# spcl/gemm_hls

Measured on AMD Instinct MI355X. Metric: GFLOP/s, fp32 GEMM N=K=M=16384 per MI355X (tiled outer-product C=A.B), and % of fp32 MFMA peak, higher is better.
Workload: dtype f32; 1 GPU; float 16384x16384x16384 (Multiply,Add) on 1 MI355X; BASELINE configs[1]; kernel=mfma_f32_256x256x16_w8_flush4096, rows_total=16384, rows_per_gpu=16384

## Files before the change

gemm_hls_amd/csrc/mm_capi.hip:

```cpp
#include <algorithm>
#include <atomic>
#include <chrono>
#include <cstdarg>
#include <cstdio>
#include <cstdlib>
#include <cstring>
#include <mutex>
#include <random>
#include <unordered_map>
#include <vector>

#include "mm_common.h"

namespace {

thread_local char g_error[512] = "";

int fail(int code, const char *fmt, ...) {
  va_list ap;
  va_start(ap, fmt);
  vsnprintf(g_error, sizeof(g_error), fmt, ap);
  va_end(ap);
  return code;
}
// ... 6 lines not shown
#define MM_HIP(call)                                   \
  do {                                                 \
    hipError_t e_ = (call);                            \
    if (e_ != hipSuccess) return hip_fail(e_, #call);  \
  } while (0)

std::once_flag g_init_once;
int g_device_count = 0;
int g_device_cus[64] = {};
int g_init_status = MM_ERR_NO_DEVICE;
char g_init_error[512] = "";

void init_once() {
  auto init_fail = [](const char *fmt, auto... args) {
    snprintf(g_init_error, sizeof(g_init_error), fmt, args...);
    g_device_count = 0;
    g_init_status = MM_ERR_NO_DEVICE;
  };
  int n = 0;
  hipError_t e = hipGetDeviceCount(&n);
  if (e != hipSuccess || n <= 0)
    return init_fail("hipGetDeviceCount: %s; this library needs an MI355X (gfx950), there is no CPU fallback",
                     e == hipSuccess ? "0 devices" : hipGetErrorString(e));
  for (int d = 0; d < n; ++d) {
    hipDeviceProp_t prop;
    e = hipGetDeviceProperties(&prop, d);
    if (e != hipSuccess) return init_fail("hipGetDeviceProperties(%d): %s", d, hipGetErrorString(e));
    if (strncmp(prop.gcnArchName, "gfx950", 6) != 0)
      return init_fail("device %d is %s; the kernels in this library are built for gfx950 only "
                       "(hide other devices with HIP_VISIBLE_DEVICES)", d, prop.gcnArchName);
    if (d < 64) g_device_cus[d] = prop.multiProcessorCount;
  }
  g_device_count = n;
  g_init_status = MM_OK;
}

int ensure_init() {
  std::call_once(g_init_once, init_once);
  return g_init_status == MM_OK ? MM_OK : fail(g_init_status, "%s", g_init_error);
}

std::mutex g_default_cfg_mutex;
mm_config_t g_default_cfg = {MM_DTYPE_F32, MM_OP_MULTIPLY, MM_OP_ADD, MM_PATH_AUTO, MM_A_ROW_MAJOR};
mm_config_t default_cfg() {
  std::lock_guard<std::mutex> lock(g_default_cfg_mutex);
  return g_default_cfg;
}

std::once_flag g_tuning_once;
std::atomic<int> g_tuning[mm::TUNE_COUNT];
const char *const kTuneName[mm::TUNE_COUNT] = {"f32_variant", "f64_variant", "f16_variant", "i8_variant", "band_rows",
                                               "valu_variant", "split_variant", "f32_splitk", "ablations", "debug_poison", "kxn_prepass_min_m",
                                               "md_virtual_devices", "ordered_variant", "half_contract", "batch_chunk",
                                               "closure_block", "lse_variant"};
const char *const kTuneEnv[mm::TUNE_COUNT] = {"MM_F32_VARIANT", "MM_F64_VARIANT", "MM_F16_VARIANT", "MM_I8_VARIANT",
                                              "MM_BAND_ROWS", "MM_VALU_VARIANT", "MM_SPLIT_VARIANT", "MM_F32_SPLITK", "MM_ABLATIONS", "MM_DEBUG_POISON", "MM_KXN_PREPASS_MIN_M",
                                              "MM_MD_VIRTUAL_DEVICES", "MM_ORDERED_VARIANT", "MM_HALF_CONTRACT", "MM_BATCH_CHUNK",
                                              "MM_CLOSURE_BLOCK", "MM_LSE_VARIANT"};
void tuning_init() {
  for (int i = 0; i < mm::TUNE_COUNT; ++i) {
    const char *e = getenv(kTuneEnv[i]);
    int v = (e && *e) ? atoi(e) : -1;
    if (i == mm::TUNE_HALF_CONTRACT && e && *e) {
      if (strcmp(e, "reference") == 0) v = 1;
      else if (strcmp(e, "wide") == 0) v = 0;
    }
    g_tuning[i].store(v, std::memory_order_relaxed);
  }
}

int check_device(int device) {
  int rc = ensure_init();
  if (rc) return rc;
  if (device < 0 || device >= g_device_count)
    return fail(MM_ERR_BAD_ARGUMENT, "device %d out of range [0, %d)", device, g_device_count);
  return MM_OK;
}

bool valid_cfg(const mm_config_t *cfg) {
  return cfg && cfg->dtype >= MM_DTYPE_F32 && cfg->dtype <= MM_DTYPE_U64 && cfg->map_op >= MM_OP_ADD &&
         cfg->map_op <= MM_OP_MAX && cfg->reduce_op >= MM_OP_ADD && cfg->reduce_op <= MM_OP_MAX &&
         (cfg->path == MM_PATH_AUTO || cfg->path == MM_PATH_ORDERED || cfg->path == MM_PATH_SPLIT) &&
         (cfg->layout_a == MM_A_ROW_MAJOR || cfg->layout_a == MM_A_TRANSPOSED);
}

int f32_variant() { return mm::tuning(mm::TUNE_F32_VARIANT); }
int f32_variant_for(const mm::Problem &p) { return mm::mfma_f32_resolve(p, f32_variant()); }

enum Family { FAM_ORDERED, FAM_ORDERED_TILE, FAM_VALU_TILE, FAM_MFMA_F32, FAM_MFMA_F64, FAM_MFMA_F16, FAM_MFMA_I8, FAM_HALF_WIDE,
              FAM_F32_SPLIT, FAM_NONE };

Family choose(const mm_config_t &cfg, const mm::Problem &slab) {
  mm::Problem p = slab;
  if (slab.n_total) { p.n = slab.n_total; p.n_total = 0; }
  const bool mul_add = cfg.map_op == MM_OP_MULTIPLY && cfg.reduce_op == MM_OP_ADD;
  const bool reference_half = cfg.path == MM_PATH_AUTO && mul_add && cfg.dtype == MM_DTYPE_F16 && mm::tuning(mm::TUNE_HALF_CONTRACT) == 1;
  if (cfg.path == MM_PATH_ORDERED || reference_half)
    return mm::tuning(mm::TUNE_ORDERED_VARIANT) != 0 && mm::valu_tile_serves(cfg, p) ? FAM_ORDERED_TILE : FAM_ORDERED;
  if (cfg.path == MM_PATH_SPLIT)
    return mul_add && cfg.dtype == MM_DTYPE_F32 && mm::mfma_f32_split_serves(p) ? FAM_F32_SPLIT : FAM_NONE;
  if (mul_add && cfg.dtype == MM_DTYPE_F32 && mm::mfma_f32_serves(p)) return FAM_MFMA_F32;
  if (mul_add && cfg.dtype == MM_DTYPE_F64 && mm::mfma_f64_serves(p)) return FAM_MFMA_F64;
  if (mul_add && cfg.dtype == MM_DTYPE_F16) return mm::mfma_f16_serves(p) ? FAM_MFMA_F16 : FAM_HALF_WIDE;
  if (mul_add && (cfg.dtype == MM_DTYPE_I8 || cfg.dtype == MM_DTYPE_U8) && mm::mfma_i8_serves(p)) return FAM_MFMA_I8;
  return mm::valu_tile_serves(cfg, p) ? FAM_VALU_TILE : FAM_ORDERED;
}

bool aligned16(const mm::Problem &p) {
  return (((uintptr_t)p.a | (uintptr_t)p.b | (uintptr_t)p.c) & 15u) == 0;
}

// ... 1478 lines not shown
```

gemm_hls_amd/csrc/mm_common.h:

```cpp
#pragma once
#include <hip/hip_runtime.h>
#include <stdint.h>
#include <stdlib.h>

#include <type_traits>

#include "../../include/mm_gemm.h"

namespace mm {

using half_t = _Float16;

template <typename T> struct Limits;
template <> struct Limits<float> {
  __host__ __device__ static constexpr float max() { return 3.40282346638528859812e+38f; }
  __host__ __device__ static constexpr float lowest() { return -3.40282346638528859812e+38f; }
};
template <> struct Limits<double> {
  __host__ __device__ static constexpr double max() { return 1.79769313486231570815e+308; }
  __host__ __device__ static constexpr double lowest() { return -1.79769313486231570815e+308; }
};
template <> struct Limits<half_t> {
  __host__ __device__ static constexpr half_t max() { return (half_t)65504.0f; }
  __host__ __device__ static constexpr half_t lowest() { return (half_t)-65504.0f; }
// ... 208 lines not shown
  switch (op) {
#define MM_CASE(OP) \
  case OP:          \
    if constexpr (OPS::template has<OP>) return f(std::integral_constant<int, OP>{}); else break;
    MM_CASE(MM_OP_ADD)
    MM_CASE(MM_OP_MULTIPLY)
    MM_CASE(MM_OP_AND)
    MM_CASE(MM_OP_MIN)
    MM_CASE(MM_OP_MAX)
#undef MM_CASE
  }
  return kErrNotSupported;
}

template <typename TYPES, typename MAPS, typename REDS, typename Fn>
int switch_config(const mm_config_t &cfg, Fn f) {
  return switch_dtype<TYPES>(cfg.dtype, [&](auto t) {
    return switch_op<MAPS>(cfg.map_op, [&](auto map) {
      return switch_op<REDS>(cfg.reduce_op, [&](auto red) { return f(t, map, red); });
    });
  });
}

inline int ensure_dynamic_lds(const void *func, int bytes, unsigned long long &mask) {
  int dev = 0;
  hipError_t e = hipGetDevice(&dev);
  if (e != hipSuccess) return (int)e;
  const unsigned long long bit = 1ull << (dev & 63);
  if (__atomic_load_n(&mask, __ATOMIC_ACQUIRE) & bit) return 0;
  e = hipFuncSetAttribute(func, hipFuncAttributeMaxDynamicSharedMemorySize, bytes);
  if (e != hipSuccess) return (int)e;
  __atomic_fetch_or(&mask, bit, __ATOMIC_RELEASE);
  return 0;
}

enum Tunable {
  TUNE_F32_VARIANT = 0,
  TUNE_F64_VARIANT,
  TUNE_F16_VARIANT,
  TUNE_I8_VARIANT,
  TUNE_BAND_ROWS,
  TUNE_VALU_VARIANT,
  TUNE_SPLIT_VARIANT,
  TUNE_F32_SPLITK,
  TUNE_ABLATIONS,
  TUNE_DEBUG_POISON,
  TUNE_KXN_PREPASS_MIN_M,
  TUNE_MD_VIRTUAL_DEVICES,
  TUNE_ORDERED_VARIANT,
  TUNE_HALF_CONTRACT,
  TUNE_BATCH_CHUNK,
  TUNE_CLOSURE_BLOCK,
  TUNE_LSE_VARIANT,
  TUNE_COUNT
};
int tuning(Tunable t);

inline unsigned band_rows(unsigned bm = 256, unsigned bn = 256, unsigned per_cu = 1) {
  const int v = tuning(TUNE_BAND_ROWS);
  if (v > 0) return (unsigned)v;
  const unsigned t = 32u * per_cu;
  unsigned best = 4, cost = ~0u;
  for (unsigned r = 1; r <= t; r *= 2) {
    const unsigned c = r * bm + (t / r) * bn;
    if (c < cost) { cost = c; best = r; }
  }
  return best;
}

struct TileCandidate { int id; unsigned bm, bn, per_cu; double eff; };
inline int pick_tile(const TileCandidate *cands, int count, unsigned n, unsigned m, double *best_time = nullptr,
                     unsigned long long copies = 1) {
  double best = 0;
  int pick = cands[0].id;
  for (int i = 0; i < count; ++i) {
    const TileCandidate &c = cands[i];
    const unsigned long long tiles = (unsigned long long)((n + c.bm - 1) / c.bm) * ((m + c.bn - 1) / c.bn) * copies;
    const unsigned long long slots = 256ull * c.per_cu, full = tiles / slots, rem = tiles % slots;
    const double t = ((double)full * c.per_cu + (double)((rem + 255) / 256)) * c.bm * c.bn / c.eff;
    if (best == 0 || t < best * 0.999) { best = t; pick = c.id; }
  }
  if (best_time) *best_time = best;
  return pick;
}

__device__ __forceinline__ unsigned xcd_remap(unsigned bid, unsigned nwg) {
  constexpr unsigned kXcds = 8;
  const unsigned q = nwg / kXcds, r = nwg % kXcds;
  const unsigned xcd = bid % kXcds, slot = bid / kXcds;
  const unsigned base = xcd < r ? xcd * (q + 1) : r * (q + 1) + (xcd - r) * q;
  return base + slot;
}

enum class Form { Single, Batched, Seeded };

template <Form F, typename G, auto KERN, typename T, typename CT>
int launch_tile(hipStream_t s, const Problem &p) {
  const unsigned tiles_n = (p.n + G::BM - 1) / G::BM, tiles_m = (p.m + G::BN - 1) / G::BN;
  static unsigned long long configured = 0;
  if (int e = ensure_dynamic_lds((const void *)KERN, G::LDS_BYTES, configured)) return e;
  hipLaunchKernelGGL(KERN, dim3(tiles_n * tiles_m * (F == Form::Single ? 1u : p.batch)), dim3(G::THREADS), G::LDS_BYTES, s,
                     (const T *)p.a, (const T *)p.b, (CT *)p.c, p.n, p.k, p.m, tiles_n, tiles_m, band_rows(G::BM, G::BN, 1),
                     F == Form::Single ? 1u : p.batch, p.stride_a, p.stride_b, p.stride_c);
  return (int)hipGetLastError();
}

// ... 64 lines not shown
```

gemm_hls_amd/csrc/mm_mfma_f32.hip:

```cpp
#include <cstdlib>
#include <type_traits>

#include "mm_common.h"

namespace mm {
namespace {

#include "mm_mfma_f32_tile.inc"
#include "mm_mfma_f32_small.inc"
#include "mm_mfma_f32_streamk.inc"

__global__ __launch_bounds__(256) void splitk_reduce_kernel(const float *__restrict__ partials, float *__restrict__ C,
                                                            size_t quads, unsigned splits) {
  const size_t i = (size_t)blockIdx.x * 256 + threadIdx.x;
  if (i >= quads) return;
  const f32x4 *src = (const f32x4 *)partials;
  f32x4 acc = src[i];
  for (unsigned s = 1; s < splits; ++s) acc += src[(size_t)s * quads + i];
  ((f32x4 *)C)[i] = acc;
}

template <typename G, bool AT = false>
int launch_geo(hipStream_t s, const Problem &p, unsigned splits = 1) {
  const unsigned tiles_n = (p.n + G::BM - 1) / G::BM, tiles_m = (p.m + G::BN - 1) / G::BN;
  static unsigned long long configured = 0;
  if (int e = ensure_dynamic_lds((const void *)mfma_f32_kernel<G, AT>, G::LDS_BYTES, configured)) return e;
  (void)hipGetLastError();
  if (splits <= 1) {
    hipLaunchKernelGGL((mfma_f32_kernel<G, AT>), dim3(tiles_n * tiles_m), dim3(G::THREADS), G::LDS_BYTES, s,
                       (const float *)p.a, (const float *)p.b, (float *)p.c, p.n, p.k, p.m, tiles_n, tiles_m,
                       band_rows(G::BM, G::BN, G::MIN_WAVES), 0u, (float *)nullptr);
    return (int)hipGetLastError();
  }
  const unsigned chunk = ((p.k + splits - 1) / splits + 31u) & ~31u;
  const size_t plane = (size_t)p.n * p.m;
  int dev = 0;
  hipError_t e = hipGetDevice(&dev);
  if (e != hipSuccess) return (int)e;
  hipMemPool_t pool = nullptr;
  if (int rc = workspace_pool(dev, &pool)) return rc;
  float *ws = nullptr;
  if ((e = hipMallocFromPoolAsync((void **)&ws, plane * splits * sizeof(float), pool, s)) != hipSuccess) return (int)e;
  hipLaunchKernelGGL((mfma_f32_kernel<G, AT>), dim3(tiles_n * tiles_m * splits), dim3(G::THREADS), G::LDS_BYTES, s,
                     (const float *)p.a, (const float *)p.b, (float *)p.c, p.n, p.k, p.m, tiles_n, tiles_m,
                     band_rows(G::BM, G::BN, G::MIN_WAVES), chunk, ws);
  int rc = (int)hipGetLastError();
  if (rc == 0) {
    const size_t quads = plane / 4;
    hipLaunchKernelGGL(splitk_reduce_kernel, dim3((unsigned)((quads + 255) / 256)), dim3(256), 0, s, ws, (float *)p.c, quads, splits);
    rc = (int)hipGetLastError();
  }
  const hipError_t f = hipFreeAsync(ws, s);
  return rc ? rc : (int)f;
}

template <typename G, bool AT, bool SEED>
__global__ __launch_bounds__(G::THREADS, G::MIN_WAVES) void mfma_f32_batched_kernel(
    const float *__restrict__ A, const float *__restrict__ B, float *__restrict__ C, unsigned N, unsigned K, unsigned M,
    unsigned tiles_n, unsigned tiles_m, unsigned kBand, unsigned batch, size_t stride_a, size_t stride_b, size_t stride_c) {
  const unsigned lin = batched_tile(A, B, C, tiles_n * tiles_m, batch, stride_a, stride_b, stride_c);
  const unsigned band = lin / (kBand * tiles_m), within = lin % (kBand * tiles_m);
  const unsigned rows_in_band = min(kBand, tiles_n - band * kBand);
  const unsigned tile_row = band * kBand + within % rows_in_band;
  const unsigned tile_col = within / rows_in_band;
  tile_body<G, AT, false, SEED>(A, B, C, N, K, M, K, M, N, M, tile_row * G::BM, tile_col * G::BN);
}

template <typename G, bool AT, bool SEED>
int launch_geo_batched_seed(hipStream_t s, const Problem &p) {
  const unsigned tiles_n = (p.n + G::BM - 1) / G::BM, tiles_m = (p.m + G::BN - 1) / G::BN;
  static unsigned long long configured = 0;
  (void)hipGetLastError();
  if (int e = ensure_dynamic_lds((const void *)mfma_f32_batched_kernel<G, AT, SEED>, G::LDS_BYTES, configured)) return e;
  hipLaunchKernelGGL((mfma_f32_batched_kernel<G, AT, SEED>), dim3(tiles_n * tiles_m * p.batch), dim3(G::THREADS), G::LDS_BYTES,
                     s, (const float *)p.a, (const float *)p.b, (float *)p.c, p.n, p.k, p.m, tiles_n, tiles_m,
                     band_rows(G::BM, G::BN, G::MIN_WAVES), p.batch, p.stride_a, p.stride_b, p.stride_c);
  return (int)hipGetLastError();
}

template <typename G, bool AT = false>
int launch_geo_batched(hipStream_t s, const Problem &p) {
  return p.seed ? launch_geo_batched_seed<G, AT, true>(s, p) : launch_geo_batched_seed<G, AT, false>(s, p);
}

using T128x256 = Geo<2, 2, 2, 16, Chain::FlushIntoC, 256, Reads::Pipelined, Dma::ScalarBase>;
using T128x256v = Geo<2, 2, 2, 16, Chain::FlushIntoC, 256, Reads::Pipelined, Dma::VectorAddress>;
using T256x256 = Geo<2, 4, 2, 16, Chain::FlushIntoC, 256, Reads::Pipelined, Dma::ScalarBase>;
using T256x256v = Geo<2, 4, 2, 16, Chain::FlushIntoC, 256, Reads::Pipelined, Dma::VectorAddress>;
using T128x128 = Geo<1, 4, 1, 32, Chain::FlushIntoC, 128, Reads::Pipelined, Dma::ScalarBase>;
using T128x128v = Geo<1, 4, 1, 32, Chain::FlushIntoC, 128, Reads::Pipelined, Dma::VectorAddress>;
using X128x256x32_2lvl = Geo<2, 2, 2, 32, Chain::TwoLevel, 16, Reads::CompilerPlaced, Dma::VectorAddress>;
using X256x256_single = Geo<2, 4, 2, 16, Chain::Single, 1, Reads::CompilerPlaced, Dma::VectorAddress>;

struct VariantInfo { int id; const char *name; unsigned bm, bn, bk, waves; };
template <typename G> constexpr VariantInfo info_of(int id, const char *name) { return {id, name, G::BM, G::BN, G::BK, G::NW}; }
constexpr VariantInfo kVariants[] = {
    info_of<T128x256>(33, "mfma_f32_128x256x16_w4x2_flush4096"),
    info_of<T256x256>(8, "mfma_f32_256x256x16_w8_flush4096"),
    info_of<T128x128>(35, "mfma_f32_128x128x32_w4x2_flush4096"),
    info_of<Small>(64, "mfma_f32_64x64x32_w4x2_flush4096"),
    info_of<X128x256x32_2lvl>(0, "mfma_f32_128x256x32_w4_2lvl"),
    info_of<X256x256_single>(3, "mfma_f32_256x256x16_w8"),
};

const VariantInfo *find_variant(int v) {
  for (const VariantInfo &i : kVariants)
    if (i.id == v) return &i;
  return nullptr;
}

}

int mfma_f32_num_variants() { return (int)(sizeof(kVariants) / sizeof(kVariants[0])); }
int mfma_f32_variant_id(int index) { return index >= 0 && index < mfma_f32_num_variants() ? kVariants[index].id : -1; }

static const TileCandidate kAutoCands[] = {{33, 128, 256, 2, 1.00}, {8, 256, 256, 1, 0.991}, {35, 128, 128, 2, 0.993}};

static bool streamk_wins(const Problem &p) {
  if (p.a_transposed || p.k % 32 != 0 || p.k < 256 || p.n_total) return false;
  if ((unsigned long long)((p.n + 127) / 128) * ((p.m + 127) / 128) * (p.k / 32) >= (1ull << 31)) return false;
  const double tiles = (double)((p.n + 127) / 128) * ((p.m + 127) / 128);
  const unsigned tn = (p.n + 127) / 128, tm = (p.m + 127) / 128;
  const bool teams_4x4 = tn % 4 == 0 && tm % 4 == 0;
  if (tiles <= 256 || tiles > (teams_4x4 ? 4096 : 2304)) return false;
  double whole = 0;
  pick_tile(kAutoCands, 3, p.n, p.m, &whole);
  const double sk = (2.0 * tiles / 512 + 0.25) * 128 * 128 / 0.993;
  return sk < 0.99 * whole;
}

template <typename G>
static int launch_small(hipStream_t s, const Problem &p, unsigned splits) {
  const unsigned tiles_n = (p.n + G::BM - 1) / G::BM, tiles_m = (p.m + G::BN - 1) / G::BN;
  static unsigned long long configured = 0;
  if (int e = ensure_dynamic_lds((const void *)mfma_f32_small_kernel<G>, G::LDS_BYTES, configured)) return e;
  (void)hipGetLastError();
  const unsigned kband = band_rows(G::BM, G::BN, G::PER_CU);
  if (splits <= 1) {
    hipLaunchKernelGGL((mfma_f32_small_kernel<G>), dim3(tiles_n * tiles_m), dim3(G::THREADS), G::LDS_BYTES, s, (const float *)p.a,
                       (const float *)p.b, (float *)p.c, p.n, p.k, p.m, tiles_n, tiles_m, kband, 0u, (float *)nullptr);
// ... 243 lines not shown
```

gemm_hls_amd/csrc/mm_mfma_f32_tile.inc:

```

using f32x4 = __attribute__((ext_vector_type(4))) float;
using f32x16 = __attribute__((ext_vector_type(16))) float;
typedef const __attribute__((address_space(1))) void *gptr_t;
typedef __attribute__((address_space(3))) void *lptr_t;

enum class Chain { Single, TwoLevel, FlushIntoC };
enum class Reads { CompilerPlaced, Pipelined };
enum class Dma { VectorAddress, ScalarBase };

template <int TM_, int WM_, int WN_, int BK_, Chain CHAIN_, int CHUNK_, Reads READS_, Dma DMA_>
struct Geo {
  static constexpr Chain CHAIN = CHAIN_;
  static constexpr Reads READS = READS_;
  static constexpr Dma DMA = DMA_;
  static constexpr int CHUNK = CHUNK_;
  static constexpr int TM = TM_, WM = WM_, WN = WN_, BK = BK_, NS = 2;
  static constexpr int TN = 4;
  static constexpr int NW = WM * WN;
  static constexpr int THREADS = NW * 64;
  static constexpr int BM = WM * TM * 32, BN = WN * 128;
  static constexpr int CPR = BK / 4;
  static constexpr int SWZ_SHIFT = (CPR == 4) ? 2 : 1;
  static constexpr int A_BYTES = BM * BK * 4, B_BYTES = BK * BN * 4;
  static constexpr int STAGE_BYTES = A_BYTES + B_BYTES;
  static constexpr int LDS_BYTES = NS * STAGE_BYTES;
  static constexpr int MIN_WAVES =
      (NW == 4 && 2 * LDS_BYTES <= 160 * 1024 && (CHAIN_ == Chain::TwoLevel ? 2 : 1) * TM * TN * 16 <= 128) ? 2 : 1;
  static constexpr int NA = A_BYTES / 1024, NB = B_BYTES / 1024;
  static constexpr int LA = NA / NW, LB = NB / NW;
  static constexpr int KG = BK / 8;
  static_assert(BK == 16 || BK == 32, "BK");
  static_assert(NA % NW == 0 && NB % NW == 0, "DMA instructions must split evenly over waves");
  static_assert(LDS_BYTES <= 160 * 1024, "LDS");
  static_assert(DMA_ == Dma::VectorAddress || READS_ == Reads::Pipelined, "the scalar-base DMA pieces are placed by hand");
};

template <typename G, bool AT, bool AGENT_STORES = false, bool SEED = false>
__device__ __forceinline__ void tile_body(const float *__restrict__ A, const float *__restrict__ B, float *__restrict__ Cst,
                                          unsigned N, unsigned K, unsigned M, unsigned lda, unsigned ldc, unsigned Nst,
                                          unsigned Mst, unsigned row0, unsigned col0) {
  constexpr int TM = G::TM, TN = G::TN, BK = G::BK, NS = G::NS, CPR = G::CPR;
  constexpr bool TWO_LEVEL = G::CHAIN == Chain::TwoLevel, FLUSH = G::CHAIN == Chain::FlushIntoC;
  constexpr bool PIPELINED = G::READS == Reads::Pipelined, SDMA = G::DMA == Dma::ScalarBase;
  extern __shared__ __attribute__((aligned(16))) char smem[];
  static_assert(!AGENT_STORES || G::TM == 1, "agent-scope stores are wired into the predicated write-back only");
  auto store_quad = [](f32x4 *dst, f32x4 v) {
    if constexpr (AGENT_STORES) asm volatile("global_store_dwordx4 %0, %1, off sc1\n\ts_nop 1" ::"v"(dst), "v"(v) : "memory");
    else *dst = v;
  };

  const unsigned lane = threadIdx.x & 63u;
  const unsigned wave = __builtin_amdgcn_readfirstlane(threadIdx.x >> 6);
  const unsigned wm = wave / G::WN, wn = wave % G::WN;
  const unsigned lo = lane & 31u, hi = lane >> 5;

  size_t a_row_off[G::LA];
  unsigned a_kchunk[G::LA];
#pragma unroll
  for (int i = 0; i < G::LA; ++i) {
    const unsigned slot = (wave + G::NW * i) * 64 + lane;
    if (AT) {
      a_kchunk[i] = slot / (G::BM / 4);
      a_row_off[i] = min(row0 + (slot % (G::BM / 4)) * 4, N - 4);
    } else {
      const unsigned row = slot / CPR, pc = slot % CPR;
      a_kchunk[i] = pc ^ ((row >> G::SWZ_SHIFT) & (CPR - 1));
      a_row_off[i] = (size_t)min(row0 + row, N - 1) * lda;
    }
  }
  unsigned b_krow[G::LB];
  unsigned b_col[G::LB];
#pragma unroll
  for (int i = 0; i < G::LB; ++i) {
    const unsigned slot = (wave + G::NW * i) * 64 + lane;
    b_krow[i] = slot / (G::BN / 4);
    b_col[i] = min(col0 + (slot % (G::BN / 4)) * 4, M - 4);
  }

  auto stage = [&](unsigned buf, unsigned k0) {
    char *base = smem + buf * G::STAGE_BYTES;
#pragma unroll
    for (int i = 0; i < G::LA; ++i) {
      const float *src;
      if (AT) src = A + (size_t)min(k0 + a_kchunk[i], K - 1) * N + a_row_off[i];
      else src = A + a_row_off[i] + min(k0 + a_kchunk[i] * 4, K - 4);
      __builtin_amdgcn_global_load_lds((gptr_t)src, (lptr_t)(base + (wave + G::NW * i) * 1024), 16, 0, 0);
    }
#pragma unroll
    for (int i = 0; i < G::LB; ++i) {
      const unsigned kr = min(k0 + b_krow[i], K - 1);
      const float *src = B + (size_t)kr * M + b_col[i];
      __builtin_amdgcn_global_load_lds((gptr_t)src, (lptr_t)(base + G::A_BYTES + (wave + G::NW * i) * 1024), 16, 0, 0);
    }
// ... 64 lines not shown
        for (int mi = 0; mi < TM; ++mi) af[mi][p] = v[mi];
      }
    } else {
#pragma unroll
      for (int mi = 0; mi < TM; ++mi)
        af[mi] = *(const f32x4 *)(base + a_frag_base + mi * 32 * (BK * 4) + achunk);
    }
#pragma unroll
    for (int p = 0; p < 4; ++p)
      bf[p] = *(const f32x4 *)(base + b_frag_base + (kg * 8 + p) * (G::BN * 4));
  };

  auto mfma_group = [&](const f32x4 (&af)[TM], const f32x4 (&bf)[4]) {
#pragma unroll
    for (int p = 0; p < 4; ++p)
#pragma unroll
      for (int mi = 0; mi < TM; ++mi)
#pragma unroll
        for (int t = 0; t < TN; ++t)
          acc[mi][t] = __builtin_amdgcn_mfma_f32_32x32x2f32(af[mi][p], bf[p][t], acc[mi][t], 0, 0, 0);
  };

  typedef __attribute__((address_space(1))) f32x4 *gquad_t;
  const bool interior_block = col0 + wn * 128 + 128 <= Mst && row0 + wm * TM * 32 + TM * 32 <= Nst &&
                              (unsigned long long)(TM * 32) * ldc * 4ull < (1ull << 32);
  auto rmw_interior = [&](bool accumulate, auto batchc, auto value) {
    constexpr int BATCH = decltype(batchc)::value;
    unsigned Mv = ldc;
    asm volatile("" : "+s"(Mv));
    char *base = (char *)(Cst + (size_t)(row0 + wm * TM * 32) * Mv + col0 + wn * 128);
    const unsigned lane_off = ((AT ? TM * 4 * hi : 4 * hi) * Mv + 4 * lo) * 4u;
#pragma unroll
    for (int mi = 0; mi < TM; ++mi)
#pragma unroll
      for (int r0 = 0; r0 < 16; r0 += BATCH) {
        f32x4 old[BATCH];
#pragma unroll
        for (int j = 0; j < BATCH; ++j) {
          const int r = r0 + j, ri = (r & 3) + 8 * (r >> 2), lrow = AT ? TM * ri + mi : mi * 32 + ri;
          old[j] = accumulate ? *(gquad_t)(base + (lane_off + (unsigned)lrow * Mv * 4u)) : (f32x4)0.0f;
        }
#pragma unroll
        for (int j = 0; j < BATCH; ++j) {
          const int r = r0 + j, ri = (r & 3) + 8 * (r >> 2), lrow = AT ? TM * ri + mi : mi * 32 + ri;
          f32x4 v;
#pragma unroll
          for (int tt = 0; tt < TN; ++tt) v[tt] = value(mi, tt, r);
          *(gquad_t)(base + (lane_off + (unsigned)lrow * Mv * 4u)) = v + old[j];
        }
        __builtin_amdgcn_sched_barrier(0);
      }
  };

  auto flush_tile = [&](bool accumulate) {
    if (PIPELINED && TM >= 2 && interior_block) {
      rmw_interior(accumulate, std::integral_constant<int, 4>{}, [&](int mi, int tt, int r) { return acc[mi][tt][r]; });
#pragma unroll
      for (int mi = 0; mi < TM; ++mi)
#pragma unroll
        for (int tt = 0; tt < TN; ++tt) acc[mi][tt] = (f32x16)0.0f;
      return;
    }
    const unsigned ccol = col0 + wn * 128 + 4 * lo;
    unsigned ldv = ldc;
    asm volatile("" : "+s"(ldv));
#pragma unroll
    for (int mi = 0; mi < TM; ++mi) {
#pragma unroll
      for (int r = 0; r < 16; ++r) {
        const unsigned ri = (r & 3) + 8 * (r >> 2) + 4 * hi;
        const unsigned row = row0 + wm * TM * 32 + (AT ? TM * ri + mi : mi * 32 + ri);
        if (ccol < Mst && row < Nst) {
          f32x4 *dst = (f32x4 *)(Cst + (size_t)row * ldv + ccol);
          f32x4 v;
#pragma unroll
          for (int tt = 0; tt < TN; ++tt) v[tt] = acc[mi][tt][r];
          if (accumulate) v += *dst;
          store_quad(dst, v);
        }
      }
#pragma unroll
      for (int tt = 0; tt < TN; ++tt) acc[mi][tt] = (f32x16)0.0f;
    }
  };

  const unsigned num_tiles = (K + BK - 1) / BK;
  constexpr int L = G::LA + G::LB;

#pragma unroll
  for (int s = 0; s < NS; ++s) stage_any(s, s * BK);
  asm volatile("s_waitcnt vmcnt(%0)" ::"n"((NS - 1) * L) : "memory");
  __builtin_amdgcn_s_barrier();

  f32x4 af0[TM], bf0[4], af1[TM], bf1[4];
  load_frags(0, 0, af0, bf0);

  auto mfma_half = [&](const f32x4 (&af)[TM], const f32x4 (&bf)[4], int h) {
#pragma unroll
    for (int p = 2 * h; p < 2 * h + 2; ++p)
#pragma unroll
      for (int mi = 0; mi < TM; ++mi)
#pragma unroll
        for (int t = 0; t < TN; ++t)
          acc[mi][t] = __builtin_amdgcn_mfma_f32_32x32x2f32(af[mi][p], bf[p][t], acc[mi][t], 0, 0, 0);
  };
  auto slab = [&](unsigned t) {
    const unsigned buf = t % NS;
#pragma unroll
    for (int kg = 0; kg < G::KG; ++kg) {
      f32x4(&afc)[TM] = (kg & 1) ? af1 : af0;
      f32x4(&bfc)[4] = (kg & 1) ? bf1 : bf0;
      f32x4(&afn)[TM] = (kg & 1) ? af0 : af1;
      f32x4(&bfn)[4] = (kg & 1) ? bf0 : bf1;
      if (PIPELINED) {
        constexpr int NM = 8 * TM, NR = TM + 4;
        constexpr bool EARLY = L + NR > NM;
        static_assert(L + NR <= 2 * NM, "a k-group has too few MFMAs to spread the DMA pieces and reads over");
        __builtin_amdgcn_sched_barrier(0);
        if (kg + 1 < G::KG) {
          mfma_half(afc, bfc, 0);
          __builtin_amdgcn_sched_barrier(0);
          load_frags(buf, kg + 1, afn, bfn);
          __builtin_amdgcn_sched_barrier(0);
          mfma_half(afc, bfc, 1);
        } else {
          if (!EARLY) {
            mfma_half(afc, bfc, 0);
            __builtin_amdgcn_sched_barrier(0);
          }
          asm volatile("s_waitcnt vmcnt(%0) lgkmcnt(0)" ::"n"((NS - 2) * L) : "memory");
          __builtin_amdgcn_s_barrier();
          __builtin_amdgcn_sched_barrier(0);
          if constexpr (SDMA) {
            constexpr int TOTAL = (EARLY ? 2 : 1) * NM, P0 = EARLY ? 0 : 2;
            auto mfma_one = [&](int idx) {
              const int p = P0 + idx / (TM * TN), mi = (idx / TN) % TM, tt = idx % TN;
              acc[mi][tt] = __builtin_amdgcn_mfma_f32_32x32x2f32(afc[mi][p], bfc[p][tt], acc[mi][tt], 0, 0, 0);
            };
#pragma unroll
            for (int i = 0; i < L; ++i) {
              mfma_one(i);
              dma_piece_s(buf, (t + NS) * BK, i);
              __builtin_amdgcn_sched_barrier(0);
            }
            load_frags((t + 1) % NS, 0, afn, bfn);
#pragma unroll
            for (int i = L; i < TOTAL; ++i) mfma_one(i);
#pragma unroll
            for (int i = 0; i < NR; ++i) {
              __builtin_amdgcn_sched_group_barrier(0x008, 1, 0);
              __builtin_amdgcn_sched_group_barrier(0x100, 1, 0);
            }
            __builtin_amdgcn_sched_group_barrier(0x008, TOTAL - L - NR, 0);
            __builtin_amdgcn_sched_barrier(0);
            continue;
          }
          stage(buf, (t + NS) * BK);
          load_frags((t + 1) % NS, 0, afn, bfn);
          if (EARLY) mfma_half(afc, bfc, 0);
          mfma_half(afc, bfc, 1);
#pragma unroll
          for (int i = 0; i < L; ++i) {
            __builtin_amdgcn_sched_group_barrier(0x008, 1, 0);
            __builtin_amdgcn_sched_group_barrier(0x020, 1, 0);
          }
#pragma unroll
          for (int i = 0; i < NR; ++i) {
            __builtin_amdgcn_sched_group_barrier(0x008, 1, 0);
            __builtin_amdgcn_sched_group_barrier(0x100, 1, 0);
          }
          __builtin_amdgcn_sched_group_barrier(0x008, (EARLY ? 2 : 1) * NM - L - NR, 0);
        }
        __builtin_amdgcn_sched_barrier(0);
        continue;
      }
      if (kg + 1 < G::KG) {
        load_frags(buf, kg + 1, afn, bfn);
      } else {
        asm volatile("s_waitcnt vmcnt(%0) lgkmcnt(0)" ::"n"((NS - 2) * L) : "memory");
        __builtin_amdgcn_s_barrier();
        stage(buf, (t + NS) * BK);
        load_frags((t + 1) % NS, 0, afn, bfn);
      }
      mfma_group(afc, bfc);
    }
  };

  const unsigned steady = num_tiles - 1;
  static_assert(!SEED || FLUSH, "the seed enters through the flush into C");
  bool flushed = SEED;
  if (FLUSH) {
    for (unsigned t0 = 0; t0 < steady; t0 += G::CHUNK) {
      const unsigned tend = min(t0 + (unsigned)G::CHUNK, steady);
      for (unsigned t = t0; t < tend; ++t) slab(t);
      if (tend < steady && K > tend * BK + 32) {
        asm volatile("s_waitcnt vmcnt(0)" ::: "memory");
        flush_tile(flushed);
        asm volatile("s_waitcnt vmcnt(0)" ::: "memory");
        flushed = true;
      }
    }
  } else if (TWO_LEVEL) {
    for (unsigned t0 = 0; t0 < steady; t0 += G::CHUNK) {
      const unsigned tend = min(t0 + (unsigned)G::CHUNK, steady);
      for (unsigned t = t0; t < tend; ++t) slab(t);
#pragma unroll
      for (int mi = 0; mi < TM; ++mi)
#pragma unroll
        for (int tt = 0; tt < TN; ++tt) {
          master[mi][tt] += acc[mi][tt];
          acc[mi][tt] = (f32x16)0.0f;
        }
    }
  } else {
    for (unsigned t = 0; t < steady; ++t) slab(t);
  }

  {
    const unsigned t = num_tiles - 1;
    const int groups = (int)((K - t * BK) / 8);
    const int shift = SDMA ? G::KG - groups : 0;
    for (int kg = 0; kg < groups; ++kg) {
      load_frags(t % NS, kg + shift, af0, bf0);
      mfma_group(af0, bf0);
    }
  }

  asm volatile("s_waitcnt vmcnt(0)" ::: "memory");

  auto write_tile = [&](bool accumulate) {
    if (PIPELINED && TM >= 2 && interior_block) {
      rmw_interior(accumulate, std::integral_constant<int, (TM * TN > 8 ? 4 : 8)>{}, [&](int mi, int tt, int r) {
        float x = acc[mi][tt][r];
        if (TWO_LEVEL) x += master[mi][tt][r];
        return x;
      });
      return;
    }
    const unsigned ccol = col0 + wn * 128 + 4 * lo;
    if (ccol < Mst) {
#pragma unroll
      for (int mi = 0; mi < TM; ++mi) {
#pragma unroll
        for (int r = 0; r < 16; ++r) {
          const unsigned ri = (r & 3) + 8 * (r >> 2) + 4 * hi;
          const unsigned row = row0 + wm * TM * 32 + (AT ? TM * ri + mi : mi * 32 + ri);
          if (row < Nst) {
            f32x4 *dst = (f32x4 *)(Cst + (size_t)row * ldc + ccol);
            f32x4 v;
#pragma unroll
            for (int tt = 0; tt < TN; ++tt) {
              float x = acc[mi][tt][r];
              if (TWO_LEVEL) x += master[mi][tt][r];
              v[tt] = x;
            }
            if (accumulate) v += *dst;
            store_quad(dst, v);
          }
        }
      }
    }
  };
  if (FLUSH && flushed) write_tile(true); else write_tile(false);
}

template <typename G, bool AT>
__global__ __launch_bounds__(G::THREADS, G::MIN_WAVES) void mfma_f32_kernel(const float *__restrict__ A,
                                                              const float *__restrict__ B,
                                                              float *__restrict__ C, unsigned N,
                                                              unsigned K, unsigned M,
                                                              unsigned tiles_n, unsigned tiles_m,
                                                              unsigned kBand, unsigned kChunk, float *__restrict__ partials) {
  const unsigned nwg = tiles_n * tiles_m;
  const unsigned lda = K;
  unsigned bid = blockIdx.x;
  if (kChunk) {
    const unsigned split = bid / nwg;
    bid -= split * nwg;
    const unsigned kbeg = split * kChunk;
    A += AT ? (size_t)kbeg * N : (size_t)kbeg;
    B += (size_t)kbeg * M;
    C = partials + (size_t)split * N * M;
    K = min(kChunk, K - kbeg);
  }
  const unsigned lin = xcd_remap(bid, nwg);
  const unsigned band = lin / (kBand * tiles_m), within = lin % (kBand * tiles_m);
  const unsigned rows_in_band = min(kBand, tiles_n - band * kBand);
  const unsigned tile_row = band * kBand + within % rows_in_band;
  const unsigned tile_col = within / rows_in_band;
  tile_body<G, AT>(A, B, C, N, K, M, lda, M, N, M, tile_row * G::BM, tile_col * G::BN);
}
```

Before: 149,500 GFLOP/s.

## Prefetch C tiles into LDS staging during final slabs before flush RMW

Adds a staged-LDS flush mode for the 256x256 fp32 MFMA tile geometry. It enlarges the LDS allocation with per-wave staging slots. The old C values are then pulled in with global_load_lds DMAs issued between MFMAs in the last slabs before each flush-into-C and the final write. The read-modify-write of C then reads from LDS and overlaps further C prefetches, instead of waiting on global loads. This aims to hide the latency of the periodic C flushes, at the cost of extra LDS footprint, more hand-placed scheduling code, and possible interference with the MFMA pipeline.

After: 149,700 GFLOP/s (median of 2 runs). Within noise of the previous version (+0.1%).

```diff
diff --git a/gemm_hls_amd/csrc/mm_capi.hip b/gemm_hls_amd/csrc/mm_capi.hip
--- a/gemm_hls_amd/csrc/mm_capi.hip
+++ b/gemm_hls_amd/csrc/mm_capi.hip
@@ -82,11 +82,11 @@
 const char *const kTuneName[mm::TUNE_COUNT] = {"f32_variant", "f64_variant", "f16_variant", "i8_variant", "band_rows",
                                                "valu_variant", "split_variant", "f32_splitk", "ablations", "debug_poison", "kxn_prepass_min_m",
                                                "md_virtual_devices", "ordered_variant", "half_contract", "batch_chunk",
-                                               "closure_block", "lse_variant"};
+                                               "closure_block", "lse_variant", "f32_flush_staging"};
 const char *const kTuneEnv[mm::TUNE_COUNT] = {"MM_F32_VARIANT", "MM_F64_VARIANT", "MM_F16_VARIANT", "MM_I8_VARIANT",
                                               "MM_BAND_ROWS", "MM_VALU_VARIANT", "MM_SPLIT_VARIANT", "MM_F32_SPLITK", "MM_ABLATIONS", "MM_DEBUG_POISON", "MM_KXN_PREPASS_MIN_M",
                                               "MM_MD_VIRTUAL_DEVICES", "MM_ORDERED_VARIANT", "MM_HALF_CONTRACT", "MM_BATCH_CHUNK",
-                                              "MM_CLOSURE_BLOCK", "MM_LSE_VARIANT"};
+                                              "MM_CLOSURE_BLOCK", "MM_LSE_VARIANT", "MM_F32_FLUSH_STAGING"};
 void tuning_init() {
   for (int i = 0; i < mm::TUNE_COUNT; ++i) {
     const char *e = getenv(kTuneEnv[i]);
diff --git a/gemm_hls_amd/csrc/mm_common.h b/gemm_hls_amd/csrc/mm_common.h
--- a/gemm_hls_amd/csrc/mm_common.h
+++ b/gemm_hls_amd/csrc/mm_common.h
@@ -284,6 +284,7 @@
   TUNE_BATCH_CHUNK,
   TUNE_CLOSURE_BLOCK,
   TUNE_LSE_VARIANT,
+  TUNE_F32_FLUSH_STAGING,
   TUNE_COUNT
 };
 int tuning(Tunable t);
diff --git a/gemm_hls_amd/csrc/mm_mfma_f32.hip b/gemm_hls_amd/csrc/mm_mfma_f32.hip
--- a/gemm_hls_amd/csrc/mm_mfma_f32.hip
+++ b/gemm_hls_amd/csrc/mm_mfma_f32.hip
@@ -19,6 +19,8 @@
   for (unsigned s = 1; s < splits; ++s) acc += src[(size_t)s * quads + i];
   ((f32x4 *)C)[i] = acc;
 }
+
+static unsigned flush_staging() { return tuning(TUNE_F32_FLUSH_STAGING) != 0 ? 1u : 0u; }
 
 template <typename G, bool AT = false>
 int launch_geo(hipStream_t s, const Problem &p, unsigned splits = 1) {
@@ -29,7 +31,7 @@
   if (splits <= 1) {
     hipLaunchKernelGGL((mfma_f32_kernel<G, AT>), dim3(tiles_n * tiles_m), dim3(G::THREADS), G::LDS_BYTES, s,
                        (const float *)p.a, (const float *)p.b, (float *)p.c, p.n, p.k, p.m, tiles_n, tiles_m,
-                       band_rows(G::BM, G::BN, G::MIN_WAVES), 0u, (float *)nullptr);
+                       band_rows(G::BM, G::BN, G::MIN_WAVES), 0u, (float *)nullptr, flush_staging());
     return (int)hipGetLastError();
   }
   const unsigned chunk = ((p.k + splits - 1) / splits + 31u) & ~31u;
@@ -43,7 +45,7 @@
   if ((e = hipMallocFromPoolAsync((void **)&ws, plane * splits * sizeof(float), pool, s)) != hipSuccess) return (int)e;
   hipLaunchKernelGGL((mfma_f32_kernel<G, AT>), dim3(tiles_n * tiles_m * splits), dim3(G::THREADS), G::LDS_BYTES, s,
                      (const float *)p.a, (const float *)p.b, (float *)p.c, p.n, p.k, p.m, tiles_n, tiles_m,
-                     band_rows(G::BM, G::BN, G::MIN_WAVES), chunk, ws);
+                     band_rows(G::BM, G::BN, G::MIN_WAVES), chunk, ws, flush_staging());
   int rc = (int)hipGetLastError();
   if (rc == 0) {
     const size_t quads = plane / 4;
@@ -57,13 +59,14 @@
 template <typename G, bool AT, bool SEED>
 __global__ __launch_bounds__(G::THREADS, G::MIN_WAVES) void mfma_f32_batched_kernel(
     const float *__restrict__ A, const float *__restrict__ B, float *__restrict__ C, unsigned N, unsigned K, unsigned M,
-    unsigned tiles_n, unsigned tiles_m, unsigned kBand, unsigned batch, size_t stride_a, size_t stride_b, size_t stride_c) {
+    unsigned tiles_n, unsigned tiles_m, unsigned kBand, unsigned batch, size_t stride_a, size_t stride_b, size_t stride_c,
+    unsigned staging) {
   const unsigned lin = batched_tile(A, B, C, tiles_n * tiles_m, batch, stride_a, stride_b, stride_c);
   const unsigned band = lin / (kBand * tiles_m), within = lin % (kBand * tiles_m);
   const unsigned rows_in_band = min(kBand, tiles_n - band * kBand);
   const unsigned tile_row = band * kBand + within % rows_in_band;
   const unsigned tile_col = within / rows_in_band;
-  tile_body<G, AT, false, SEED>(A, B, C, N, K, M, K, M, N, M, tile_row * G::BM, tile_col * G::BN);
+  tile_body<G, AT, false, SEED>(A, B, C, N, K, M, K, M, N, M, tile_row * G::BM, tile_col * G::BN, staging != 0);
 }
 
 template <typename G, bool AT, bool SEED>
@@ -74,7 +77,7 @@
   if (int e = ensure_dynamic_lds((const void *)mfma_f32_batched_kernel<G, AT, SEED>, G::LDS_BYTES, configured)) return e;
   hipLaunchKernelGGL((mfma_f32_batched_kernel<G, AT, SEED>), dim3(tiles_n * tiles_m * p.batch), dim3(G::THREADS), G::LDS_BYTES,
                      s, (const float *)p.a, (const float *)p.b, (float *)p.c, p.n, p.k, p.m, tiles_n, tiles_m,
-                     band_rows(G::BM, G::BN, G::MIN_WAVES), p.batch, p.stride_a, p.stride_b, p.stride_c);
+                     band_rows(G::BM, G::BN, G::MIN_WAVES), p.batch, p.stride_a, p.stride_b, p.stride_c, flush_staging());
   return (int)hipGetLastError();
 }
 
@@ -85,7 +88,7 @@
 
 using T128x256 = Geo<2, 2, 2, 16, Chain::FlushIntoC, 256, Reads::Pipelined, Dma::ScalarBase>;
 using T128x256v = Geo<2, 2, 2, 16, Chain::FlushIntoC, 256, Reads::Pipelined, Dma::VectorAddress>;
-using T256x256 = Geo<2, 4, 2, 16, Chain::FlushIntoC, 256, Reads::Pipelined, Dma::ScalarBase>;
+using T256x256 = Geo<2, 4, 2, 16, Chain::FlushIntoC, 256, Reads::Pipelined, Dma::ScalarBase, Flush::StagedLds>;
 using T256x256v = Geo<2, 4, 2, 16, Chain::FlushIntoC, 256, Reads::Pipelined, Dma::VectorAddress>;
 using T128x128 = Geo<1, 4, 1, 32, Chain::FlushIntoC, 128, Reads::Pipelined, Dma::ScalarBase>;
 using T128x128v = Geo<1, 4, 1, 32, Chain::FlushIntoC, 128, Reads::Pipelined, Dma::VectorAddress>;
diff --git a/gemm_hls_amd/csrc/mm_mfma_f32_tile.inc b/gemm_hls_amd/csrc/mm_mfma_f32_tile.inc
--- a/gemm_hls_amd/csrc/mm_mfma_f32_tile.inc
+++ b/gemm_hls_amd/csrc/mm_mfma_f32_tile.inc
@@ -7,9 +7,11 @@
 enum class Chain { Single, TwoLevel, FlushIntoC };
 enum class Reads { CompilerPlaced, Pipelined };
 enum class Dma { VectorAddress, ScalarBase };
-
-template <int TM_, int WM_, int WN_, int BK_, Chain CHAIN_, int CHUNK_, Reads READS_, Dma DMA_>
+enum class Flush { Direct, StagedLds };
+
+template <int TM_, int WM_, int WN_, int BK_, Chain CHAIN_, int CHUNK_, Reads READS_, Dma DMA_, Flush FLUSH_ = Flush::Direct>
 struct Geo {
+  static constexpr Flush FLUSH = FLUSH_;
   static constexpr Chain CHAIN = CHAIN_;
   static constexpr Reads READS = READS_;
   static constexpr Dma DMA = DMA_;
@@ -23,7 +25,10 @@
   static constexpr int SWZ_SHIFT = (CPR == 4) ? 2 : 1;
   static constexpr int A_BYTES = BM * BK * 4, B_BYTES = BK * BN * 4;
   static constexpr int STAGE_BYTES = A_BYTES + B_BYTES;
-  static constexpr int LDS_BYTES = NS * STAGE_BYTES;
+  static constexpr int RING_BYTES = NS * STAGE_BYTES;
+  static constexpr int STAGING_SLOTS = 12;
+  static constexpr int STAGING_BYTES = FLUSH_ == Flush::StagedLds ? WM_ * WN_ * STAGING_SLOTS * 1024 : 0;
+  static constexpr int LDS_BYTES = RING_BYTES + STAGING_BYTES;
   static constexpr int MIN_WAVES =
       (NW == 4 && 2 * LDS_BYTES <= 160 * 1024 && (CHAIN_ == Chain::TwoLevel ? 2 : 1) * TM * TN * 16 <= 128) ? 2 : 1;
   static constexpr int NA = A_BYTES / 1024, NB = B_BYTES / 1024;
@@ -33,12 +38,14 @@
   static_assert(NA % NW == 0 && NB % NW == 0, "DMA instructions must split evenly over waves");
   static_assert(LDS_BYTES <= 160 * 1024, "LDS");
   static_assert(DMA_ == Dma::VectorAddress || READS_ == Reads::Pipelined, "the scalar-base DMA pieces are placed by hand");
+  static_assert(FLUSH_ == Flush::Direct || (CHAIN_ == Chain::FlushIntoC && DMA_ == Dma::ScalarBase && TM_ == 2 && BK_ == 16),
+                "the staged flush is written for the scalar-base 64-row wavefront block with two k-groups per slab");
 };
 
 template <typename G, bool AT, bool AGENT_STORES = false, bool SEED = false>
 __device__ __forceinline__ void tile_body(const float *__restrict__ A, const float *__restrict__ B, float *__restrict__ Cst,
                                           unsigned N, unsigned K, unsigned M, unsigned lda, unsigned ldc, unsigned Nst,
-                                          unsigned Mst, unsigned row0, unsigned col0) {
+                                          unsigned Mst, unsigned row0, unsigned col0, bool staging = false) {
   constexpr int TM = G::TM, TN = G::TN, BK = G::BK, NS = G::NS, CPR = G::CPR;
   constexpr bool TWO_LEVEL = G::CHAIN == Chain::TwoLevel, FLUSH = G::CHAIN == Chain::FlushIntoC;
   constexpr bool PIPELINED = G::READS == Reads::Pipelined, SDMA = G::DMA == Dma::ScalarBase;
@@ -209,7 +216,74 @@
       }
   };
 
+  constexpr bool STAGED_GEO = G::FLUSH == Flush::StagedLds;
+  constexpr int SLOTS = G::STAGING_SLOTS, ACCESSES = 16 * TM;
+  const bool staged = STAGED_GEO && staging && interior_block;
+  bool prefetched = false;
+  auto c_dma = [&](int i, int slot) {
+    const int mi = i / 16, r = i % 16, ri = (r & 3) + 8 * (r >> 2), lrow = AT ? TM * ri + mi : mi * 32 + ri;
+    unsigned Mv = ldc;
+    asm volatile("" : "+s"(Mv));
+    unsigned long long base = (unsigned long long)(Cst + (size_t)(row0 + wm * TM * 32 + lrow) * Mv + col0 + wn * 128);
+    const unsigned blo = __builtin_amdgcn_readfirstlane((unsigned)base), bhi = __builtin_amdgcn_readfirstlane((unsigned)(base >> 32));
+    base = ((unsigned long long)bhi << 32) | blo;
+    const unsigned vo = ((AT ? TM * 4 * hi : 4 * hi) * Mv + 4 * lo) * 4u;
+    const unsigned la = lds_base + G::RING_BYTES + (wave * SLOTS + slot) * 1024;
+    unsigned keep;
+    asm volatile("s_mov_b32 %0, m0\n\ts_mov_b32 m0, %3\n\ts_nop 0\n\tglobal_load_lds_dwordx4 %1, %2\n\ts_mov_b32 m0, %0"
+                 : "=&s"(keep) : "v"(vo), "s"(base), "s"(la) : "memory");
+  };
+  auto staged_rmw = [&](auto value) {
+    constexpr int BATCH = 4;
+    static_assert(SLOTS % BATCH == 0 && ACCESSES % BATCH == 0, "whole batches");
+    unsigned Mv = ldc;
+    asm volatile("" : "+s"(Mv));
+    char *base = (char *)(Cst + (size_t)(row0 + wm * TM * 32) * Mv + col0 + wn * 128);
+    const unsigned lane_off = ((AT ? TM * 4 * hi : 4 * hi) * Mv + 4 * lo) * 4u;
+    const char *mine = smem + G::RING_BYTES + wave * (SLOTS * 1024) + lane * 16;
+    if (!prefetched) {
+#pragma unroll
+      for (int j = 0; j < SLOTS; ++j) c_dma(j, j);
+    }
+    prefetched = false;
+    asm volatile("s_waitcnt vmcnt(0)" ::: "memory");
+#pragma unroll
+    for (int i0 = 0; i0 < ACCESSES; i0 += BATCH) {
+      if (i0 > 0 && i0 % SLOTS == 0) asm volatile("s_waitcnt vmcnt(0)" ::: "memory");
+      f32x4 old[BATCH];
+#pragma unroll
+      for (int j = 0; j < BATCH; ++j) old[j] = *(const f32x4 *)(mine + ((i0 + j) % SLOTS) * 1024);
+      asm volatile("s_waitcnt lgkmcnt(0)" ::: "memory");
+#pragma unroll
+      for (int j = 0; j < BATCH; ++j) asm volatile("" : "+v"(old[j]));
+      __builtin_amdgcn_sched_barrier(0);
+#pragma unroll
+      for (int j = 0; j < BATCH; ++j)
+        if (i0 + j + SLOTS < ACCESSES) c_dma(i0 + j + SLOTS, (i0 + j) % SLOTS);
+      __builtin_amdgcn_sched_barrier(0);
+#pragma unroll
+      for (int j = 0; j < BATCH; ++j) {
+        const int i = i0 + j, mi = i / 16, r = i % 16, ri = (r & 3) + 8 * (r >> 2), lrow = AT ? TM * ri + mi : mi * 32 + ri;
+        f32x4 v;
+#pragma unroll
+        for (int tt = 0; tt < TN; ++tt) v[tt] = value(mi, tt, r);
+        *(gquad_t)(base + (lane_off + (unsigned)lrow * Mv * 4u)) = v + old[j];
+      }
+      __builtin_amdgcn_sched_barrier(0);
+    }
+  };
+
   auto flush_tile = [&](bool accumulate) {
+    if constexpr (STAGED_GEO) {
+      if (staged && accumulate) {
+        staged_rmw([&](int mi, int tt, int r) { return acc[mi][tt][r]; });
+#pragma unroll
+        for (int mi = 0; mi < TM; ++mi)
+#pragma unroll
+          for (int tt = 0; tt < TN; ++tt) acc[mi][tt] = (f32x16)0.0f;
+        return;
+      }
+    }
     if (PIPELINED && TM >= 2 && interior_block) {
       rmw_interior(accumulate, std::integral_constant<int, 4>{}, [&](int mi, int tt, int r) { return acc[mi][tt][r]; });
 #pragma unroll
@@ -261,7 +335,10 @@
         for (int t = 0; t < TN; ++t)
           acc[mi][t] = __builtin_amdgcn_mfma_f32_32x32x2f32(af[mi][p], bf[p][t], acc[mi][t], 0, 0, 0);
   };
-  auto slab = [&](unsigned t) {
+  constexpr int PF_PER_SLAB = 3, PF_SLABS = SLOTS / PF_PER_SLAB;
+  using NoPf = std::integral_constant<int, -1>;
+  auto slab = [&](unsigned t, auto pfc) {
+    constexpr int PF = decltype(pfc)::value;
     const unsigned buf = t % NS;
 #pragma unroll
     for (int kg = 0; kg < G::KG; ++kg) {
@@ -279,7 +356,19 @@
           __builtin_amdgcn_sched_barrier(0);
           load_frags(buf, kg + 1, afn, bfn);
           __builtin_amdgcn_sched_barrier(0);
-          mfma_half(afc, bfc, 1);
+          if constexpr (PF >= 0) {
+#pragma unroll
+            for (int i = 0; i < NM; ++i) {
+              const int p = 2 + i / (TM * TN), mi = (i / TN) % TM, tt = i % TN;
+              acc[mi][tt] = __builtin_amdgcn_mfma_f32_32x32x2f32(afc[mi][p], bfc[p][tt], acc[mi][tt], 0, 0, 0);
+              if (kg == 0 && i < PF_PER_SLAB) {
+                c_dma(PF + i, PF + i);
+                __builtin_amdgcn_sched_barrier(0);
+              }
+            }
+          } else {
+            mfma_half(afc, bfc, 1);
+          }
         } else {
           if (!EARLY) {
             mfma_half(afc, bfc, 0);
@@ -349,7 +438,23 @@
   if (FLUSH) {
     for (unsigned t0 = 0; t0 < steady; t0 += G::CHUNK) {
       const unsigned tend = min(t0 + (unsigned)G::CHUNK, steady);
-      for (unsigned t = t0; t < tend; ++t) slab(t);
+      if constexpr (STAGED_GEO) {
+        const bool flush_follows = tend < steady && K > tend * BK + 32;
+        unsigned tpf = tend;
+        if (staged && flushed && (flush_follows || tend == steady) && tend - t0 > (unsigned)PF_SLABS) tpf = tend - 1 - PF_SLABS;
+        for (unsigned t = t0; t < tpf; ++t) slab(t, NoPf{});
+        if (tpf < tend) {
+          static_assert(PF_SLABS == 4, "one call per prefetching slab");
+          slab(tpf, std::integral_constant<int, 0>{});
+          slab(tpf + 1, std::integral_constant<int, PF_PER_SLAB>{});
+          slab(tpf + 2, std::integral_constant<int, 2 * PF_PER_SLAB>{});
+          slab(tpf + 3, std::integral_constant<int, 3 * PF_PER_SLAB>{});
+          slab(tpf + 4, NoPf{});
+          prefetched = true;
+        }
+      } else {
+        for (unsigned t = t0; t < tend; ++t) slab(t, NoPf{});
+      }
       if (tend < steady && K > tend * BK + 32) {
         asm volatile("s_waitcnt vmcnt(0)" ::: "memory");
         flush_tile(flushed);
@@ -360,7 +465,7 @@
   } else if (TWO_LEVEL) {
     for (unsigned t0 = 0; t0 < steady; t0 += G::CHUNK) {
       const unsigned tend = min(t0 + (unsigned)G::CHUNK, steady);
-      for (unsigned t = t0; t < tend; ++t) slab(t);
+      for (unsigned t = t0; t < tend; ++t) slab(t, NoPf{});
 #pragma unroll
       for (int mi = 0; mi < TM; ++mi)
 #pragma unroll
@@ -370,7 +475,7 @@
         }
     }
   } else {
-    for (unsigned t = 0; t < steady; ++t) slab(t);
+    for (unsigned t = 0; t < steady; ++t) slab(t, NoPf{});
   }
 
   {
@@ -386,6 +491,12 @@
   asm volatile("s_waitcnt vmcnt(0)" ::: "memory");
 
   auto write_tile = [&](bool accumulate) {
+    if constexpr (STAGED_GEO) {
+      if (staged && accumulate) {
+        staged_rmw([&](int mi, int tt, int r) { return acc[mi][tt][r]; });
+        return;
+      }
+    }
     if (PIPELINED && TM >= 2 && interior_block) {
       rmw_interior(accumulate, std::integral_constant<int, (TM * TN > 8 ? 4 : 8)>{}, [&](int mi, int tt, int r) {
         float x = acc[mi][tt][r];
@@ -427,7 +538,8 @@
                                                               float *__restrict__ C, unsigned N,
                                                               unsigned K, unsigned M,
                                                               unsigned tiles_n, unsigned tiles_m,
-                                                              unsigned kBand, unsigned kChunk, float *__restrict__ partials) {
+                                                              unsigned kBand, unsigned kChunk, float *__restrict__ partials,
+                                                              unsigned staging) {
   const unsigned nwg = tiles_n * tiles_m;
   const unsigned lda = K;
   unsigned bid = blockIdx.x;
@@ -445,5 +557,5 @@
   const unsigned rows_in_band = min(kBand, tiles_n - band * kBand);
   const unsigned tile_row = band * kBand + within % rows_in_band;
   const unsigned tile_col = within / rows_in_band;
-  tile_body<G, AT>(A, B, C, N, K, M, lda, M, N, M, tile_row * G::BM, tile_col * G::BN);
+  tile_body<G, AT>(A, B, C, N, K, M, lda, M, N, M, tile_row * G::BM, tile_col * G::BN, staging != 0);
 }
```
